# myshell-ai/OpenVoice

Measured on NVIDIA H100. Metric: audio_seconds_per_second, higher is better.
Workload: dtype f32 (3xFP16 split-precision tensor-core convs with fp32 accumulation, fp32 FFMA elsewhere)

## Files before the change

### include/ovc.h

```cpp
#ifndef OVC_B200_H
#define OVC_B200_H

#include <stddef.h>
#include <stdint.h>

#ifdef __cplusplus
extern "C" {
#endif

#define OVC_ABI_VERSION 17

#if defined(__GNUC__)
#define OVC_API __attribute__((visibility("default")))
#else
#define OVC_API
#endif

enum {
  OVC_OK = 0,
  OVC_ERR_INVALID = -1,
  OVC_ERR_CUDA = -2,
  OVC_ERR_STATE = -3,
  OVC_ERR_MISSING = -4,
  OVC_ERR_NOMEM = -5
};
// ... 154 lines not shown
                                      float* d_stats, int32_t* d_cum, float* d_g, int64_t* d_y_lengths, void* stream);
OVC_API int ovc_tts_decode_windows_tokens(ovc_ctx* ctx, const float* stats, const int32_t* cum, const float* g,
                                          const int64_t* y_lengths, int N, int T, const int64_t* row, const int64_t* frame0,
                                          const int64_t* len, int W, int Wmax, const uint64_t* seed, const int64_t* stream,
                                          const float* noise_scale, float* o, float* z_p, void* cuda_stream);

OVC_API int ovc_set_precision(ovc_ctx* ctx, int mode);

#define OVC_OPT_TTS_SIMPLE 2
#define OVC_OPT_GRAPH 3
#define OVC_OPT_PDL 5
#define OVC_OPT_BRANCHES 7
#define OVC_OPT_PAIR 8
#define OVC_OPT_PAIR_OCC 9
#define OVC_OPT_STAGED_EPI 10
OVC_API int ovc_set_option(ovc_ctx* ctx, int key, int value);

OVC_API int ovc_last_launch_count(const ovc_ctx* ctx);

OVC_API int ovc_graph_replays(const ovc_ctx* ctx);

OVC_API int ovc_profile_enable(ovc_ctx* ctx, int enable);
OVC_API int ovc_profile_read(ovc_ctx* ctx, double* ms, int64_t* launches, double* flops, double* bytes);
OVC_API int ovc_profile_detail(ovc_ctx* ctx, int max, char* names, double* ms, double* flops, double* bytes,
                               int* family);

OVC_API int ovc_debug_enable(ovc_ctx* ctx, int enable);
OVC_API int ovc_debug_fetch(ovc_ctx* ctx, const char* name, float* host_out, size_t max_floats,
                    int64_t* shape4 );

// ... 5 lines not shown
```

### openvoice_b200/_native.py

```python
from __future__ import annotations

import ctypes as C
import os
from typing import Dict, Iterable, Optional, Tuple

_HERE = os.path.dirname(os.path.abspath(__file__))
LIB_PATH = os.path.join(_HERE, "libovc_b200.so")

ABI_VERSION = 17
EXPORTS = (
    "ovc_abi_version", "ovc_last_error", "ovc_create", "ovc_destroy", "ovc_load_tensor",
    "ovc_finalize_weights", "ovc_workspace_floats", "ovc_voice_conversion", "ovc_last_launch_count",
    "ovc_profile_enable", "ovc_profile_read", "ovc_profile_detail", "ovc_debug_enable", "ovc_debug_fetch",
    "ovc_spectrogram", "ovc_convert_waveform", "ovc_set_precision", "ovc_reference_encoder",
    "ovc_tts_info", "ovc_tts_encode", "ovc_tts_decode", "ovc_set_option", "ovc_graph_replays",
    "ovc_reference_encoder_ragged", "ovc_resample", "ovc_resample_span", "ovc_voice_conversion_items",
    "ovc_convert_waveform_items", "ovc_tts_encode_items", "ovc_tts_decode_items", "ovc_philox_normals",
    "ovc_tts_encode_state", "ovc_tts_decode_windows", "ovc_spectrogram_ring", "ovc_splice",
    "ovc_tts_encode_state_rows", "ovc_tts_state_rows", "ovc_resample_plan", "ovc_resample_rings",
    "ovc_voice_conversion_frames", "ovc_convert_waveform_frames", "ovc_tone_track_expand",
    "ovc_tts_encode_g", "ovc_tts_encode_state_tokens", "ovc_tts_decode_windows_tokens", "ovc_tts_encode_state_rows_tokens",
    "ovc_tts_state_rows_tokens", "ovc_reference_encoder_stream", "ovc_reference_encoder_stream_state_floats",
    "ovc_generate_frames",
)
# ... 259 lines not shown
            _check(self.lib, rc, f"ovc_load_tensor({k})")
            (ignored if rc == 1 else used).append(k)
        self.finalized = False
        return used, ignored

    def finalize(self):
        _check(self.lib, self.lib.ovc_finalize_weights(self.handle), "ovc_finalize_weights")
        self.finalized = True

    def set_precision(self, mode: str):
        m = PRECISIONS[mode]
        _check(self.lib, self.lib.ovc_set_precision(self.handle, m), "ovc_set_precision")
        self.precision = mode

    def set_option(self, key: str, value: int):
        k = {"tts_simple": 2, "graph": 3, "pdl": 5, "branches": 7, "pair": 8, "pair_occ": 9, "staged_epi": 10}[key]
        _check(self.lib, self.lib.ovc_set_option(self.handle, k, int(value)), "ovc_set_option")

    def voice_conversion(self, spec, lengths, g_src, g_tgt, noise=None, tau: float = 0.3, seed: int = 0,
                         ragged: bool = False, latents: bool = True, stream=None, items: Optional[dict] = None, out=None):
        import torch
        assert spec.is_cuda and spec.dtype == torch.float32 and spec.is_contiguous()
        assert lengths.is_cuda and lengths.dtype == torch.int64 and lengths.is_contiguous()
        B, S, T = spec.shape
        gs, fs = se_arg(g_src, B, self.hp.gin_channels, T, "g_src")
        gt, ft = se_arg(g_tgt, B, self.hp.gin_channels, T, "g_tgt")
        if noise is not None:
            noise = noise.contiguous().float()
            assert tuple(noise.shape) == (B, self.hp.inter_channels, T)
        hop = self.hp.hop_length
        if out is not None:
# ... 486 lines not shown
```

### openvoice_b200/csrc/ovc_lib.cu

```cuda
#include <cuda_runtime.h>

#include <algorithm>
#include <cmath>
#include <cstdarg>
#include <cstdio>
#include <cstdlib>
#include <cstring>
#include <map>
#include <string>
#include <vector>

#include "../../include/ovc.h"
#include "ovc_convpack.h"
#include "ovc_small.cuh"
#include "ovc_tcconv.cuh"
#include "ovc_tts.cuh"
#include "ovc_refenc.cuh"
#include "ovc_resample.cuh"
#include "ovc_splice.h"
#include "ovc_variants.h"

namespace ovc {

static thread_local std::string g_err;
// ... 135 lines not shown
  WNLayers flow_wn[4];
  ConvLayer dec_pre, dec_ups[4];
  ConvLayer rb_c1[12][3], rb_c2[12][3];
  TcLayer tc_c1[12][3], tc_c2[12][3], tc_ups[4], tc_pre;
  float* d_tcw = nullptr;
  std::vector<float> h_tcw;
  int precision = 0;
  bool tts_simple = false;
  bool use_graph = true;
  int use_pdl = 2;
  bool use_branches = true;
  int par_frames = 512;
  bool use_pair = true;
  bool use_pair_occ = true;
  bool use_staged_epi = true;
  bool pair_occ2_ok[TCN_N_OCC2] = {};
  cudaStream_t br_stream[2] = {nullptr, nullptr};
  cudaEvent_t br_ev[4] = {nullptr, nullptr, nullptr, nullptr};
  size_t post_w_off = 0;
  size_t cond_w_off = 0, cond_b_off = 0;
  int* d_cond_wrow = nullptr;
  int* d_cond_sel = nullptr;
  int cond_rows_out = 0;
  int cond_off_enc = 0, cond_off_fsrc = 0, cond_off_ftgt = 0, cond_off_dec = 0;
  int cond_off_enc_tc = 0, cond_off_fsrc_tc = 0, cond_off_ftgt_tc = 0;
  int* d_cond_cols[2][3] = {};
  int cond_pf_cols[2][3] = {};
  int cond_pf_off[2][3][4] = {};

  float2* d_tw = nullptr;
// ... 427 lines not shown
  if (c->d_w) { cudaFree(c->d_w); c->d_w = nullptr; }
  c->w_floats = c->h_w.size();
  CK(cudaMalloc(&c->d_w, c->w_floats * sizeof(float)));
  CK(cudaMemcpy(c->d_w, c->h_w.data(), c->w_floats * sizeof(float), cudaMemcpyHostToDevice));
  if (c->d_tcw) { cudaFree(c->d_tcw); c->d_tcw = nullptr; }
  CK(cudaMalloc(&c->d_tcw, c->h_tcw.size() * sizeof(float)));
  CK(cudaMemcpy(c->d_tcw, c->h_tcw.data(), c->h_tcw.size() * sizeof(float), cudaMemcpyHostToDevice));
  c->h_tcw.clear();
  c->h_tcw.shrink_to_fit();
  for (int TN : {128, 64, 32})
    for (bool staged : {false, true}) {
      const TcKernel k = tc_conv_kernel(TN, staged), p = tc_pair_kernel(TN, TcPairOcc(), staged);
      CK(cudaFuncSetAttribute(k.fn, cudaFuncAttributeMaxDynamicSharedMemorySize, (int)k.smem));
      CK(cudaFuncSetAttribute(p.fn, cudaFuncAttributeMaxDynamicSharedMemorySize, (int)p.smem));
    }
  for (int i = 0; i < TCN_N_OCC2; ++i) {
    const TcKernel k = tc_pair_kernel(kTcPairOcc2[i].C, kTcPairOcc2[i].o);
    CK(cudaFuncSetAttribute(k.fn, cudaFuncAttributeMaxDynamicSharedMemorySize, (int)k.smem));
    int blocks = 0;
    CK(cudaOccupancyMaxActiveBlocksPerMultiprocessor(&blocks, k.fn, k.threads, k.smem));
    c->pair_occ2_ok[i] = blocks >= 2;
    if (blocks < 2)
      fprintf(stderr, "ovc: the C = %d conv-pair kernel with %d operand buffer(s) fits %d CTA(s) per SM, not 2; its pairs run "
              "one CTA per SM\n", kTcPairOcc2[i].C, kTcPairOcc2[i].o.nabuf, blocks);
  }
  if (c->d_cond_wrow) cudaFree(c->d_cond_wrow);
  if (c->d_cond_sel) cudaFree(c->d_cond_sel);
  CK(cudaMalloc(&c->d_cond_wrow, wrow.size() * sizeof(int)));
  CK(cudaMalloc(&c->d_cond_sel, sel.size() * sizeof(int)));
  CK(cudaMemcpy(c->d_cond_wrow, wrow.data(), wrow.size() * sizeof(int), cudaMemcpyHostToDevice));
// ... 135 lines not shown
  CK(cudaEventRecord(c->ev[c->ev_used], r.st));
  return OVC_OK;
}
static int prof_end(Run& r, int variant, int family, double flops, double bytes, int tag = 0) {
  ovc_ctx* c = r.c;
  if (!c->prof) return OVC_OK;
  CK(cudaEventRecord(c->ev[c->ev_used + 1], r.st));
  c->ev_used += 2;
  c->ev_flops.push_back(flops);
  c->ev_bytes.push_back(bytes);
  c->ev_variant.push_back(variant);
  c->ev_family.push_back(family);
  c->ev_tag.push_back(tag);
  return OVC_OK;
}
enum { V_TCPAIR128 = -14, V_TCPAIR64 = -12, V_TCPAIR32 = -13, V_TC128 = -1, V_TC64 = -2, V_TC32 = -3, V_TRANSPOSE = -4, V_TTS_DENSE = -5, V_TTS_LN = -6, V_TTS_SCORES = -7,
       V_TTS_ATTN = -8, V_TTS_DW = -9, V_TTS_SPLINE = -10, V_TTS_MISC = -11 };
static const char* variant_name(int v) {
  if (v >= 0) return kInfo[v].name;
  switch (v) {
    case V_TCPAIR128: return "PAIR_N128";
    case V_TCPAIR64: return "PAIR_N64";
    case V_TCPAIR32: return "PAIR_N32";
    case V_TC128: return "TC3_N128";
    case V_TC64: return "TC3_N64";
    case V_TC32: return "TC3_N32";
    case V_TTS_DENSE: return "TTS_DENSE32";
    case V_TTS_LN: return "TTS_LAYERNORM";
    case V_TTS_SCORES: return "TTS_SCORES";
    case V_TTS_ATTN: return "TTS_ATTN_OUT";
    case V_TTS_DW: return "TTS_DWCONV";
    case V_TTS_SPLINE: return "TTS_SPLINE";
    case V_TTS_MISC: return "TTS_MISC";
    default: return "TRANSPOSE";
  }
// ... 119 lines not shown
    TRY(launch(r, wn.in[i], a, T));
    ConvArgs b{};
    b.x = acts; b.x_bs = bs; b.x_pitch = P;
    b.bias = r.c->d_w + wn.rs[i].b_off; b.bias_bs = 0;
    b.y = x; b.y_bs = bs; b.y_pitch = P;
    b.s = skip; b.s_bs = bs; b.s_pitch = P;
    b.lens_in = r.lens; b.lens_out = r.lens; b.mul_in = 1; b.mul_out = 1;
    b.slope = 1.f;
    b.split = (i < n - 1) ? 192 : 0;
    b.flags = (i == 0) ? F_FIRST : 0;
    TRY(launch(r, wn.rs[i], b, T));
  }
  return OVC_OK;
}

static int run_wn_tc(Run& r, const WNLayers& wn, float* x, float* skip, float* acts, float* x_cl, float* skip_cl,
                     const CondRef& cond_tc) {
  const int P = r.P, T = r.Tmax;
  const int n = (int)wn.tc_in.size();
  TRY(launch_transpose(r, x, x_cl, 192, P));
  for (int i = 0; i < n; ++i) {
    TcExtra g;
    g.epi = 1; g.bias = cond_tc.p + (size_t)i * 384; g.bias_bs = cond_tc.bs; g.bias_ts = cond_tc.ts; g.y_ld = 192;
    g.use_lens_frames = true;
    TRY(launch_tc(r, wn.tc_in[i], x_cl, acts, nullptr, T, 1, 1.f, 1.f, 0, 0, g));
    TcExtra q;
    q.epi = 2; q.s = skip_cl; q.split = (i < n - 1) ? 192 : 0; q.first = (i == 0); q.y_ld = 192; q.use_lens_frames = true;
    TRY(launch_tc(r, wn.tc_rs[i], acts, x_cl, nullptr, T, 1, 1.f, 1.f, 0, 0, q));
  }
  TRY(launch_transpose(r, skip_cl, skip, P, 192));
  return OVC_OK;
}

static int run_flow(Run& r, const WsLayout& W, float* ws, bool reverse, const CondRef& cond) {
  ovc_ctx* c = r.c;
  const int P = r.P, T = r.Tmax;
// ... 103 lines not shown
  }
  e->launches = c->launches;
  CK(cudaGraphLaunch(e->exec, st));
  c->graph_replays++;
  return OVC_OK;
}

static int set_call_params(ovc_ctx* c, uint64_t seed, float tau, const ItemParams& items, cudaStream_t st) {
  if (!c->d_callp) CK(cudaMalloc(&c->d_callp, sizeof(CallParams)));
  set_call_params_kernel<<<1, 1, 0, st>>>(c->d_callp, seed, tau, items);
  CK(cudaGetLastError());
  return OVC_OK;
}
static uintptr_t option_bits(const ovc_ctx* c) {
  return (uintptr_t)c->precision | ((uintptr_t)c->use_pdl << 15) | ((uintptr_t)c->use_branches << 14) | ((uintptr_t)c->use_pair << 17) |
         ((uintptr_t)c->use_pair_occ << 18) | ((uintptr_t)c->use_staged_epi << 19);
}

static int ensure_ws(ovc_ctx* c, const WsLayout& W, int B, int Tmax, cudaStream_t st) {
  if (W.total <= c->ws_floats) return OVC_OK;
  CK(cudaStreamSynchronize(st));
  drop_graphs(c);
  if (c->d_ws) CK(cudaFree(c->d_ws));
  c->d_ws = nullptr;
  c->ws_floats = 0;
  cudaError_t e = cudaMalloc(&c->d_ws, W.total * sizeof(float));
  if (e != cudaSuccess) {
    cudaGetLastError();
    return fail(OVC_ERR_NOMEM, "workspace of %.2f GB for B=%d Tmax=%d does not fit: %s", W.total * 4e-9, B, Tmax,
                cudaGetErrorString(e));
  }
// ... 1095 lines not shown
}

int ovc_set_option(ovc_ctx* c, int key, int value) {
  if (!c) return fail(OVC_ERR_INVALID, "null context");
  switch (key) {
    case OVC_OPT_TTS_SIMPLE: c->tts_simple = value != 0; return OVC_OK;
    case OVC_OPT_GRAPH: c->use_graph = value != 0; return OVC_OK;
    case OVC_OPT_PDL:
      if (value < 0 || value > 2) return fail(OVC_ERR_INVALID, "pdl must be 0, 1 or 2");
      c->use_pdl = value;
      return OVC_OK;
    case OVC_OPT_BRANCHES: c->use_branches = value != 0; return OVC_OK;
    case OVC_OPT_PAIR: c->use_pair = value != 0; return OVC_OK;
    case OVC_OPT_PAIR_OCC: c->use_pair_occ = value != 0; return OVC_OK;
    case OVC_OPT_STAGED_EPI: c->use_staged_epi = value != 0; return OVC_OK;
    default: return fail(OVC_ERR_INVALID, "unknown option %d", key);
  }
}

int ovc_last_launch_count(const ovc_ctx* c) { return c ? c->launches : 0; }

int ovc_graph_replays(const ovc_ctx* c) { return c ? c->graph_replays : 0; }

int ovc_profile_enable(ovc_ctx* c, int enable) {
  if (!c) return fail(OVC_ERR_INVALID, "null context");
  c->prof = enable != 0;
  c->ev_used = 0;
  c->ev_flops.clear();
  c->ev_bytes.clear();
  c->ev_variant.clear();
// ... 76 lines not shown
```

### openvoice_b200/csrc/ovc_tcconv.cuh

```cuda
#pragma once
#include "ovc_conv.cuh"
#include "ovc_tc.cuh"
#include "ovc_tcpack.h"

namespace ovc {

struct TcConvArgs {
  const float* x; long long x_bs;
  const uint16_t* w;
  const float* bias; long long bias_bs;
  float* y; long long y_bs; int y_ld;
  const float* r;
  float* s; long long s_bs;
  int epi;
  int split; int first;
  const long long* lens; int tmax; int mul;
  const long long* lens_x; int has_lens_x;
  int Cin; int Ntot; int K; int DIL;
  float slope; float scale; int accumulate;
  int passes;
  const uint16_t* w2; const float* bias2;
  long long bias_ts;
};

__device__ __forceinline__ void pdl_launch_dependents() { asm volatile("griddepcontrol.launch_dependents;" ::: "memory"); }
__device__ __forceinline__ void pdl_wait() { asm volatile("griddepcontrol.wait;" ::: "memory"); }

__device__ __forceinline__ void mbar_arrive(uint64_t* bar) {
  asm volatile("mbarrier.arrive.shared::cta.b64 _, [%0];" ::"r"(smem_u32(bar)) : "memory");
}
__device__ __forceinline__ void named_bar_sync(int id, int threads) {
  asm volatile("bar.sync %0, %1;" ::"r"(id), "r"(threads) : "memory");
}
__device__ __forceinline__ void named_bar_arrive(int id, int threads) {
  asm volatile("bar.arrive %0, %1;" ::"r"(id), "r"(threads) : "memory");
}

template <int TN>
__device__ __forceinline__ float tc_result(const float (&d)[TN], bool two, int j) {
  return two ? fmaf(d[TN / 2 + j], tc::kLoInv, d[j]) : d[j];
}

template <int TN, bool PF, class V>
__device__ __forceinline__ void tc_epilogue_body(const TcConvArgs& a, V v_at, int b, int t0, int n0, int lim, int row_a) {
  const int csub = (threadIdx.x & 3) * 2;
  float* yb = a.y + (size_t)b * a.y_bs;
  const float* rb = a.r ? a.r + (size_t)b * a.y_bs : nullptr;
  float* sb = a.s ? a.s + (size_t)b * a.s_bs : nullptr;
  const int ta = t0 + row_a, tb = ta + 8;
  const bool oka = ta < lim, okb = tb < lim;
  const float* bias_a = a.bias + (size_t)b * a.bias_bs + (PF ? (size_t)min(ta, a.tmax - 1) * a.bias_ts : 0);
  const float* bias_b = a.bias + (size_t)b * a.bias_bs + (PF ? (size_t)min(tb, a.tmax - 1) * a.bias_ts : 0);
#pragma unroll
  for (int c0 = 0; c0 < TN; c0 += 32) {
    float v[16];
#pragma unroll
    for (int i = 0; i < 16; ++i) v[i] = v_at(c0 / 2 + i);
#pragma unroll
    for (int g = 0; g < 4; ++g) {
// ... 21 lines not shown
          ob.x = yc.x + ob.x; ob.y = yc.y + ob.y;
        }
        if (a.scale != 1.f) { oa.x *= a.scale; oa.y *= a.scale; ob.x *= a.scale; ob.y *= a.scale; }
        if (oka) *reinterpret_cast<float2*>(ypa + 8 * g) = oa;
        if (okb) *reinterpret_cast<float2*>(ypb + 8 * g) = ob;
      }
    } else if (a.epi == 1) {
      float* ypa = yb + (size_t)ta * a.y_ld + ((n0 + c0) >> 1) + csub;
      float* ypb = yb + (size_t)tb * a.y_ld + ((n0 + c0) >> 1) + csub;
#pragma unroll
      for (int g = 0; g < 2; ++g) {
        const float2 oa = make_float2(tanhf(v[4 * g]) * sigmoidf_acc(v[4 * (g + 2)]),
                                      tanhf(v[4 * g + 1]) * sigmoidf_acc(v[4 * (g + 2) + 1]));
        const float2 ob = make_float2(tanhf(v[4 * g + 2]) * sigmoidf_acc(v[4 * (g + 2) + 2]),
                                      tanhf(v[4 * g + 3]) * sigmoidf_acc(v[4 * (g + 2) + 3]));
        if (oka) *reinterpret_cast<float2*>(ypa + 8 * g) = oa;
        if (okb) *reinterpret_cast<float2*>(ypb + 8 * g) = ob;
      }
    } else {
      const int col = n0 + c0;
      const bool to_x = col < a.split;
      const bool add = to_x || !a.first;
      float* dst = (to_x ? yb + col : sb + (col - a.split)) + csub;
#pragma unroll
      for (int g = 0; g < 4; ++g) {
        float2 oa = make_float2(v[4 * g], v[4 * g + 1]), ob = make_float2(v[4 * g + 2], v[4 * g + 3]);
        if (add) {
          const float2 qa = oka ? *reinterpret_cast<const float2*>(dst + (size_t)ta * a.y_ld + 8 * g) : make_float2(0.f, 0.f);
          const float2 qb = okb ? *reinterpret_cast<const float2*>(dst + (size_t)tb * a.y_ld + 8 * g) : make_float2(0.f, 0.f);
          oa = make_float2(qa.x + oa.x, qa.y + oa.y);
          ob = make_float2(qb.x + ob.x, qb.y + ob.y);
        }
        if (oka) *reinterpret_cast<float2*>(dst + (size_t)ta * a.y_ld + 8 * g) = oa;
        if (okb) *reinterpret_cast<float2*>(dst + (size_t)tb * a.y_ld + 8 * g) = ob;
      }
    }
  }
}

template <int TN, class V>
__device__ __forceinline__ void tc_epilogue_v(const TcConvArgs& a, V v_at, int b, int t0, int n0, int lim, int row_a) {
  if (a.bias_ts) tc_epilogue_body<TN, true>(a, v_at, b, t0, n0, lim, row_a);
  else tc_epilogue_body<TN, false>(a, v_at, b, t0, n0, lim, row_a);
}

template <int TN>
__device__ __forceinline__ void tc_epilogue(const TcConvArgs& a, const float (&d)[TN], int b, int t0, int n0, int lim, int row_a) {
  const bool two = a.passes == 3;
  tc_epilogue_v<TN>(a, [&](int j) { return tc_result<TN>(d, two, j); }, b, t0, n0, lim, row_a);
}
__device__ __forceinline__ TcConvArgs tc_pair_epilogue_args(const TcConvArgs& a, int TN) {
  TcConvArgs e = a;
  e.y_ld = TN; e.r = a.x; e.bias = a.bias2; e.bias_bs = 0; e.bias_ts = 0; e.epi = 0;
  return e;
}

template <int TN>
__device__ __forceinline__ void tc_mma_step(float (&d)[TN], uint64_t a_hi, uint64_t a_lo, uint64_t b, bool three, bool first) {
  float (&lo)[TN / 2] = *reinterpret_cast<float(*)[TN / 2]>(&d[TN / 2]);
  float (&hi)[TN / 2] = *reinterpret_cast<float(*)[TN / 2]>(&d[0]);
  tc::Wgmma<TN>::mma(hi, a_hi, b, first ? 0 : 1);
  if (three) {
    tc::Wgmma<TN>::mma(lo, a_hi, b + TN, first ? 0 : 1);
    tc::Wgmma<TN>::mma(lo, a_lo, b, 1);
  }
}

constexpr int TCN_THREADS = 384;
constexpr int TCN_NCT = 96;

template <int TN, bool PAIR, int OCC = 1, int NAB = 2, bool STAGED = false>
struct TcnCfg {
  static_assert(!PAIR || TN == 32 || TN == 64 || TN == 128, "conv pairs: C = 32, 64 or 128");
  static_assert(OCC == 1 || (PAIR && TN <= 64), "two CTAs per SM: C = 32 / 64 pairs");
  static_assert(!STAGED || (TN == 128 && OCC == 1), "staged epilogue: TN = 128, one CTA per SM");
  static constexpr int THREADS = STAGED ? TCN_THREADS + 128 : TCN_THREADS;
  static constexpr int KCH = 32, NKC = KCH / 8;
  static constexpr int ROWS = 194;
  static constexpr int ROWS2 = TCN_ROWS2;
  static constexpr int NABUF = NAB;
  static constexpr int RING = PAIR ? tc_pair_ring(TN, OCC, NAB) : tc_ring_slots(TN, PAIR);
  static constexpr int SLOT_BYTES = 2 * 2 * TN * 16;
  static constexpr int A_BUF_BYTES = 2 * NKC * ROWS * 16;
  static constexpr int A2_BYTES = PAIR ? 2 * (TN / 8) * ROWS2 * 16 : 0;
// ... 36 lines not shown
  constexpr uint32_t BYTES = Cfg::SLOT_BYTES;

  if (tid == 0) {
    for (int i = 0; i < NABUF; ++i) { mbar_init(&a_full[i], TCN_NCT); mbar_init(&a_empty[i], 2); }
    for (int i = 0; i < RING; ++i) { mbar_init(&b_full[i], 1); mbar_init(&b_empty[i], 2); }
    if (STAGED) { mbar_init(s_full, 256); mbar_init(s_empty, 128); }
    fence_mbar_init();
  }
  if (PAIR) {
    for (int i = tid; i < Cfg::A2_BYTES / 16; i += Cfg::THREADS) reinterpret_cast<uint4*>(a2buf)[i] = make_uint4(0u, 0u, 0u, 0u);
    asm volatile("fence.proxy.async.shared::cta;" ::: "memory");
  }
  __syncthreads();
  pdl_launch_dependents();
  if (warp != 0) pdl_wait();

#define TCN_FOR_TILES                                                                                   \
  for (int tile = blockIdx.x; tile < total; tile += gridDim.x) {                                        \
    const int b = tile / n_tt, t0 = (tile % n_tt) * R;                                                  \
    const int lim = (a.lens ? (int)min((long long)a.tmax, a.lens[b]) : a.tmax) * a.mul;                 \
    const int lim_x = a.has_lens_x ? (int)min((long long)a.tmax, a.lens_x[b]) * a.mul : lim;            \
    (void)lim_x;                                                                                        \
    if (t0 >= lim) continue;

  if (warp < 4) {
    tc::regs_dealloc<Cfg::PROD_REGS>();
    if (warp == 0) {
      if (lane == 0) {
        const unsigned char* wt = reinterpret_cast<const unsigned char*>(a.w) + (size_t)blockIdx.y * n_slots * BYTES;
        if (resident) {
          for (int it = 0; it < n_w; ++it) {
            const unsigned char* src = it < n_slots ? wt + (size_t)it * BYTES
                                                    : reinterpret_cast<const unsigned char*>(a.w2) + (size_t)(it - n_slots) * BYTES;
            mbar_expect_tx(&b_full[it], BYTES);
            tma_bulk_g2s(bring + it * BYTES, src, BYTES, &b_full[it]);
          }
          for (int it = 0; it < n_w; ++it) mbar_wait(&b_full[it], 0u);
        } else {
// ... 193 lines not shown
          }
        }
        tc::wgmma_commit();
        tc::wgmma_wait<0>();
        tc::fence_regs(d);
        if (leader && prev >= 0) mbar_arrive(&b_empty[prev]);
        if constexpr (STAGED) {
          named_bar_sync(3, 256);
          stage_tile();
        } else {
          tc_epilogue<TN>(tc_pair_epilogue_args(a, TN), d, b, t0, 0, min(lim, t0 + R), row_a);
        }
      }
    }
  }
#undef TCN_FOR_TILES
}

struct TcKernel {
  void (*fn)(TcConvArgs, int, int) = nullptr;
  size_t smem = 0;
  int threads = 0;
};
using TcPairKernel = TcKernel;
template <int TN, bool PAIR, int OCC = 1, int NAB = 2, bool STAGED = false>
inline TcKernel tc_kernel() {
  using Cfg = TcnCfg<TN, PAIR, OCC, NAB, STAGED>;
  return {tcconv_kernel<TN, PAIR, OCC, NAB, STAGED>, Cfg::SMEM_BYTES, Cfg::THREADS};
}
inline bool tc_stage_pays(int K, int passes) { return passes * K >= 15; }
inline TcKernel tc_conv_kernel(int TN, bool staged) {
  if (TN == 128) return staged ? tc_kernel<128, false, 1, 2, true>() : tc_kernel<128, false>();
  if (TN == 64) return tc_kernel<64, false>();
  if (TN == 32) return tc_kernel<32, false>();
  return {};
}
inline TcKernel tc_pair_kernel(int C, TcPairOcc o, bool staged = false) {
  if (o.occ == 1 && o.nabuf == 2) {
    if (C == 128) return staged ? tc_kernel<128, true, 1, 2, true>() : tc_kernel<128, true>();
    if (C == 64) return tc_kernel<64, true>();
    if (C == 32) return tc_kernel<32, true>();
  } else if (o.occ == 2) {
    if (C == 32 && o.nabuf == 2) return tc_kernel<32, true, 2, 2>();
    if (C == 32 && o.nabuf == 1) return tc_kernel<32, true, 2, 1>();
    if (C == 64 && o.nabuf == 1) return tc_kernel<64, true, 2, 1>();
  }
  return {};
}
constexpr int TCN_N_OCC2 = 3;
constexpr struct { int C; TcPairOcc o; } kTcPairOcc2[TCN_N_OCC2] = {{32, {2, 2}}, {32, {2, 1}}, {64, {2, 1}}};

template <int C>
__global__ void __launch_bounds__(256) conv_post_cl_kernel(const float* __restrict__ x, long long x_bs,
                                                           const float* __restrict__ w, float* __restrict__ y,
                                                           long long y_bs, int y_len, const long long* lens, int tmax,
                                                           int mul) {
  constexpr int TB = 256, ROWS = TB + 6, LD = ROWS + 3;
  __shared__ float ws[7][C];
  __shared__ float xs[C][LD];
  for (int i = threadIdx.x; i < C * 7; i += blockDim.x) ws[i % 7][i / 7] = w[i];
  const int b = blockIdx.y;
// ... 47 lines not shown
```

### openvoice_b200/csrc/ovc_tcpack.h

```cpp
#pragma once
#include <cuda_fp16.h>
#include <stddef.h>
#include <stdint.h>

#include <algorithm>

namespace ovc {

constexpr int TCN_HMAX = 25;
constexpr int TCN_ROWS2 = 146;

constexpr int tc_ring_slots(int TN, bool pair) {
  return pair ? (TN == 32 ? 44 : TN == 64 ? 24 : 12) : (TN == 32 ? 22 : 12);
}

struct TcGeom {
  int Cin = 0, Ntot = 0, K = 0, DIL = 1, TN = 0;
};

inline int tc_tile_n(int Ntot, int Cin, int K, int DIL) {
  if (Ntot <= 0 || Cin <= 0 || K <= 0 || DIL <= 0) return 0;
  if (Ntot % 32 || Cin % 32 || (K - 1) / 2 * DIL > TCN_HMAX) return 0;
  return Ntot % 128 == 0 ? 128 : (Ntot % 64 == 0 ? 64 : 32);
}
// ... 41 lines not shown
}

inline bool tc_pair_fits(const TcGeom& T1, const TcGeom& T2) {
  if (!(T1.TN == 32 || T1.TN == 64)) return false;
  const int ring = tc_ring_slots(T1.TN, true);
  return T1.Ntot == T1.TN && T1.Cin == T1.TN && T2.Ntot == T1.TN && T2.Cin == T1.TN && T2.TN == T1.TN && T2.K == T1.K &&
         T2.DIL == 1 && (T1.K - 1) / 2 * T1.DIL <= TCN_HMAX && 2 * (T1.Cin / 16) * T1.K <= ring && T1.K <= 5;
}

inline bool tc_pair_fuses(const TcGeom& T1, const TcGeom& T2) {
  if (!(T1.TN == 32 || T1.TN == 64 || T1.TN == 128)) return false;
  return T1.Ntot == T1.TN && T1.Cin == T1.TN && T2.Ntot == T1.TN && T2.Cin == T1.TN && T2.TN == T1.TN && T2.K == T1.K &&
         T2.DIL == 1 && (T1.K - 1) / 2 * T1.DIL <= TCN_HMAX && 128 + 2 * ((T2.K - 1) / 2) <= TCN_ROWS2;
}

struct TcGrid {
  int n_tt = 0, total = 0, grid_x = 0, ncol = 0;
};
inline TcGrid tc_grid(int t_len, int B, int Ntot, int TN, int sm_count, int grid_div) {
  TcGrid g;
  g.n_tt = (t_len + 127) / 128;
  g.total = g.n_tt * B;
  g.ncol = Ntot / TN;
  const int per_col = std::max(1, sm_count / g.ncol / std::max(1, grid_div));
  g.grid_x = std::min(g.total, per_col);
  return g;
}
inline TcGrid tc_pair_grid(int t_len, int B, int K, int sm_count, int occ = 1) {
  TcGrid g;
  const int R = 128 - (K - 1);
// ... 30 lines not shown
```

Before: 2381.

## Fuse WaveNet gated conv and res/skip projection into one tensor-core kernel

Adds a warp-specialized kernel that computes the K=5 gate convolution for each 128-frame tile, applies tanh·sigmoid gating in the epilogue, and stores the activations as split fp16 hi/lo in shared memory. The 1x1 res/skip projection then reads those activations straight from shared memory, and the residual add reads the input buffer. This removes the global round-trip of the activation tensor and one launch per WaveNet layer, at the cost of a large shared-memory footprint that limits occupancy to one block per SM. The fused path is on by default but only runs when the tile count is at least the SM count.

```diff
diff --git a/include/ovc.h b/include/ovc.h
--- a/include/ovc.h
+++ b/include/ovc.h
@@ -8,7 +8,7 @@
 extern "C" {
 #endif
 
-#define OVC_ABI_VERSION 17
+#define OVC_ABI_VERSION 18
 
 #if defined(__GNUC__)
 #define OVC_API __attribute__((visibility("default")))
@@ -193,6 +193,7 @@
 #define OVC_OPT_PAIR 8
 #define OVC_OPT_PAIR_OCC 9
 #define OVC_OPT_STAGED_EPI 10
+#define OVC_OPT_WN_FUSE 11
 OVC_API int ovc_set_option(ovc_ctx* ctx, int key, int value);
 
 OVC_API int ovc_last_launch_count(const ovc_ctx* ctx);
diff --git a/openvoice_b200/_native.py b/openvoice_b200/_native.py
--- a/openvoice_b200/_native.py
+++ b/openvoice_b200/_native.py
@@ -7,7 +7,7 @@
 _HERE = os.path.dirname(os.path.abspath(__file__))
 LIB_PATH = os.path.join(_HERE, "libovc_b200.so")
 
-ABI_VERSION = 17
+ABI_VERSION = 18
 EXPORTS = (
     "ovc_abi_version", "ovc_last_error", "ovc_create", "ovc_destroy", "ovc_load_tensor",
     "ovc_finalize_weights", "ovc_workspace_floats", "ovc_voice_conversion", "ovc_last_launch_count",
@@ -297,7 +297,7 @@
         self.precision = mode
 
     def set_option(self, key: str, value: int):
-        k = {"tts_simple": 2, "graph": 3, "pdl": 5, "branches": 7, "pair": 8, "pair_occ": 9, "staged_epi": 10}[key]
+        k = {"tts_simple": 2, "graph": 3, "pdl": 5, "branches": 7, "pair": 8, "pair_occ": 9, "staged_epi": 10, "wn_fuse": 11}[key]
         _check(self.lib, self.lib.ovc_set_option(self.handle, k, int(value)), "ovc_set_option")
 
     def voice_conversion(self, spec, lengths, g_src, g_tgt, noise=None, tau: float = 0.3, seed: int = 0,
diff --git a/openvoice_b200/csrc/ovc_lib.cu b/openvoice_b200/csrc/ovc_lib.cu
--- a/openvoice_b200/csrc/ovc_lib.cu
+++ b/openvoice_b200/csrc/ovc_lib.cu
@@ -173,6 +173,7 @@
   bool use_pair = true;
   bool use_pair_occ = true;
   bool use_staged_epi = true;
+  bool use_wn_fuse = true;
   bool pair_occ2_ok[TCN_N_OCC2] = {};
   cudaStream_t br_stream[2] = {nullptr, nullptr};
   cudaEvent_t br_ev[4] = {nullptr, nullptr, nullptr, nullptr};
@@ -630,6 +631,10 @@
       CK(cudaFuncSetAttribute(k.fn, cudaFuncAttributeMaxDynamicSharedMemorySize, (int)k.smem));
       CK(cudaFuncSetAttribute(p.fn, cudaFuncAttributeMaxDynamicSharedMemorySize, (int)p.smem));
     }
+  for (int TN2 : {128, 64}) {
+    const TcKernel k = tc_wn_kernel(TN2);
+    CK(cudaFuncSetAttribute(k.fn, cudaFuncAttributeMaxDynamicSharedMemorySize, (int)k.smem));
+  }
   for (int i = 0; i < TCN_N_OCC2; ++i) {
     const TcKernel k = tc_pair_kernel(kTcPairOcc2[i].C, kTcPairOcc2[i].o);
     CK(cudaFuncSetAttribute(k.fn, cudaFuncAttributeMaxDynamicSharedMemorySize, (int)k.smem));
@@ -795,11 +800,12 @@
   c->ev_tag.push_back(tag);
   return OVC_OK;
 }
-enum { V_TCPAIR128 = -14, V_TCPAIR64 = -12, V_TCPAIR32 = -13, V_TC128 = -1, V_TC64 = -2, V_TC32 = -3, V_TRANSPOSE = -4, V_TTS_DENSE = -5, V_TTS_LN = -6, V_TTS_SCORES = -7,
+enum { V_TCWN = -15, V_TCPAIR128 = -14, V_TCPAIR64 = -12, V_TCPAIR32 = -13, V_TC128 = -1, V_TC64 = -2, V_TC32 = -3, V_TRANSPOSE = -4, V_TTS_DENSE = -5, V_TTS_LN = -6, V_TTS_SCORES = -7,
        V_TTS_ATTN = -8, V_TTS_DW = -9, V_TTS_SPLINE = -10, V_TTS_MISC = -11 };
 static const char* variant_name(int v) {
   if (v >= 0) return kInfo[v].name;
   switch (v) {
+    case V_TCWN: return "TCWN";
     case V_TCPAIR128: return "PAIR_N128";
     case V_TCPAIR64: return "PAIR_N64";
     case V_TCPAIR32: return "PAIR_N32";
@@ -949,12 +955,46 @@
   return OVC_OK;
 }
 
+static int launch_wn(Run& r, const TcLayer& G, const TcLayer& RS, const float* x_in, float* x_out, float* skip,
+                     const CondRef& cond, int first) {
+  const int P = r.P, T = r.Tmax;
+  TcConvArgs a{};
+  a.x = x_in; a.x_bs = 192LL * P;
+  a.w = reinterpret_cast<const uint16_t*>(r.c->d_tcw + G.w_off);
+  a.bias = cond.p; a.bias_bs = cond.bs; a.bias_ts = cond.ts;
+  a.w2 = reinterpret_cast<const uint16_t*>(r.c->d_tcw + RS.w_off); a.bias2 = r.c->d_tcw + RS.b_off;
+  a.y = x_out; a.y_bs = 192LL * P; a.y_ld = 192;
+  a.r = x_in;
+  a.s = skip; a.s_bs = a.y_bs;
+  a.split = RS.Ntot - 192; a.first = first;
+  a.lens = r.lens; a.tmax = T; a.mul = 1;
+  a.Cin = G.Cin; a.Ntot = G.Ntot; a.K = G.K; a.DIL = G.DIL;
+  a.slope = 1.f; a.scale = 1.f;
+  a.passes = r.c->precision == 2 ? 1 : 3;
+  if (!tc_wn_fuses(G, RS)) return fail(OVC_ERR_INVALID, "WaveNet layer %d -> %d / %d does not fit the fused layer kernel", G.Cin, G.Ntot, RS.Ntot);
+  const TcKernel k = tc_wn_kernel(RS.TN);
+  const TcGrid g = tc_grid(T, r.B, 128, 128, r.c->sm_count, 1);
+  TRY(prof_begin(r));
+  CK(launch_ex(k.fn, dim3((unsigned)g.grid_x, 1, 1), k.threads, k.smem, r.st, r.c->use_pdl != 0, a, g.n_tt, g.total));
+  CK(cudaGetLastError());
+  r.c->launches++;
+  const double units = (double)r.B * T;
+  TRY(prof_end(r, V_TCWN, 0, 2.0 * 192 * (G.Ntot * G.K + RS.Ntot) * units, 4.0 * 192 * (3 + (first ? 0 : 1)) * units));
+  return OVC_OK;
+}
+
 static int run_wn_tc(Run& r, const WNLayers& wn, float* x, float* skip, float* acts, float* x_cl, float* skip_cl,
                      const CondRef& cond_tc) {
   const int P = r.P, T = r.Tmax;
   const int n = (int)wn.tc_in.size();
   TRY(launch_transpose(r, x, x_cl, 192, P));
+  const bool fuse = r.c->use_wn_fuse && tc_wn_pays(tc_grid(T, r.B, 128, 128, r.c->sm_count, 1).total, r.c->sm_count);
   for (int i = 0; i < n; ++i) {
+    if (fuse) {
+      float* x_in = i % 2 ? acts : x_cl;
+      TRY(launch_wn(r, wn.tc_in[i], wn.tc_rs[i], x_in, i % 2 ? x_cl : acts, skip_cl, cond_tc.at(i * 384), i == 0));
+      continue;
+    }
     TcExtra g;
     g.epi = 1; g.bias = cond_tc.p + (size_t)i * 384; g.bias_bs = cond_tc.bs; g.bias_ts = cond_tc.ts; g.y_ld = 192;
     g.use_lens_frames = true;
@@ -1088,7 +1128,7 @@
 }
 static uintptr_t option_bits(const ovc_ctx* c) {
   return (uintptr_t)c->precision | ((uintptr_t)c->use_pdl << 15) | ((uintptr_t)c->use_branches << 14) | ((uintptr_t)c->use_pair << 17) |
-         ((uintptr_t)c->use_pair_occ << 18) | ((uintptr_t)c->use_staged_epi << 19);
+         ((uintptr_t)c->use_pair_occ << 18) | ((uintptr_t)c->use_staged_epi << 19) | ((uintptr_t)c->use_wn_fuse << 20);
 }
 
 static int ensure_ws(ovc_ctx* c, const WsLayout& W, int B, int Tmax, cudaStream_t st) {
@@ -2214,6 +2254,7 @@
     case OVC_OPT_PAIR: c->use_pair = value != 0; return OVC_OK;
     case OVC_OPT_PAIR_OCC: c->use_pair_occ = value != 0; return OVC_OK;
     case OVC_OPT_STAGED_EPI: c->use_staged_epi = value != 0; return OVC_OK;
+    case OVC_OPT_WN_FUSE: c->use_wn_fuse = value != 0; return OVC_OK;
     default: return fail(OVC_ERR_INVALID, "unknown option %d", key);
   }
 }
diff --git a/openvoice_b200/csrc/ovc_tcconv.cuh b/openvoice_b200/csrc/ovc_tcconv.cuh
--- a/openvoice_b200/csrc/ovc_tcconv.cuh
+++ b/openvoice_b200/csrc/ovc_tcconv.cuh
@@ -36,13 +36,16 @@
   asm volatile("bar.arrive %0, %1;" ::"r"(id), "r"(threads) : "memory");
 }
 
+constexpr int TCWN_ACT_HALF_BYTES = (192 / 8) * 128 * 16;
+
 template <int TN>
 __device__ __forceinline__ float tc_result(const float (&d)[TN], bool two, int j) {
   return two ? fmaf(d[TN / 2 + j], tc::kLoInv, d[j]) : d[j];
 }
 
-template <int TN, bool PF, class V>
-__device__ __forceinline__ void tc_epilogue_body(const TcConvArgs& a, V v_at, int b, int t0, int n0, int lim, int row_a) {
+template <int TN, bool PF, bool WN, class V>
+__device__ __forceinline__ void tc_epilogue_body(const TcConvArgs& a, V v_at, int b, int t0, int n0, int lim, int row_a,
+                                                 unsigned char* acts) {
   const int csub = (threadIdx.x & 3) * 2;
   float* yb = a.y + (size_t)b * a.y_bs;
   const float* rb = a.r ? a.r + (size_t)b * a.y_bs : nullptr;
@@ -94,6 +97,19 @@
                                       tanhf(v[4 * g + 1]) * sigmoidf_acc(v[4 * (g + 2) + 1]));
         const float2 ob = make_float2(tanhf(v[4 * g + 2]) * sigmoidf_acc(v[4 * (g + 2) + 2]),
                                       tanhf(v[4 * g + 3]) * sigmoidf_acc(v[4 * (g + 2) + 3]));
+        if constexpr (WN) {
+          const int off = ((((n0 + c0) >> 4) + g) * 128 + row_a) * 16 + csub * 2;
+          const float2 za = oka ? oa : make_float2(0.f, 0.f), zb = okb ? ob : make_float2(0.f, 0.f);
+          const __half2 ha = __floats2half2_rn(za.x, za.y), hb = __floats2half2_rn(zb.x, zb.y);
+          const float2 fa = __half22float2(ha), fb = __half22float2(hb);
+          *reinterpret_cast<__half2*>(acts + off) = ha;
+          *reinterpret_cast<__half2*>(acts + off + 8 * 16) = hb;
+          *reinterpret_cast<__half2*>(acts + TCWN_ACT_HALF_BYTES + off) =
+              __floats2half2_rn((za.x - fa.x) * tc::kLoScale, (za.y - fa.y) * tc::kLoScale);
+          *reinterpret_cast<__half2*>(acts + TCWN_ACT_HALF_BYTES + off + 8 * 16) =
+              __floats2half2_rn((zb.x - fb.x) * tc::kLoScale, (zb.y - fb.y) * tc::kLoScale);
+          continue;
+        }
         if (oka) *reinterpret_cast<float2*>(ypa + 8 * g) = oa;
         if (okb) *reinterpret_cast<float2*>(ypb + 8 * g) = ob;
       }
@@ -102,12 +118,13 @@
       const bool to_x = col < a.split;
       const bool add = to_x || !a.first;
       float* dst = (to_x ? yb + col : sb + (col - a.split)) + csub;
+      const float* src = WN && to_x ? rb + col + csub : dst;
 #pragma unroll
       for (int g = 0; g < 4; ++g) {
         float2 oa = make_float2(v[4 * g], v[4 * g + 1]), ob = make_float2(v[4 * g + 2], v[4 * g + 3]);
         if (add) {
-          const float2 qa = oka ? *reinterpret_cast<const float2*>(dst + (size_t)ta * a.y_ld + 8 * g) : make_float2(0.f, 0.f);
-          const float2 qb = okb ? *reinterpret_cast<const float2*>(dst + (size_t)tb * a.y_ld + 8 * g) : make_float2(0.f, 0.f);
+          const float2 qa = oka ? *reinterpret_cast<const float2*>(src + (size_t)ta * a.y_ld + 8 * g) : make_float2(0.f, 0.f);
+          const float2 qb = okb ? *reinterpret_cast<const float2*>(src + (size_t)tb * a.y_ld + 8 * g) : make_float2(0.f, 0.f);
           oa = make_float2(qa.x + oa.x, qa.y + oa.y);
           ob = make_float2(qb.x + ob.x, qb.y + ob.y);
         }
@@ -118,16 +135,18 @@
   }
 }
 
-template <int TN, class V>
-__device__ __forceinline__ void tc_epilogue_v(const TcConvArgs& a, V v_at, int b, int t0, int n0, int lim, int row_a) {
-  if (a.bias_ts) tc_epilogue_body<TN, true>(a, v_at, b, t0, n0, lim, row_a);
-  else tc_epilogue_body<TN, false>(a, v_at, b, t0, n0, lim, row_a);
-}
-
-template <int TN>
-__device__ __forceinline__ void tc_epilogue(const TcConvArgs& a, const float (&d)[TN], int b, int t0, int n0, int lim, int row_a) {
+template <int TN, bool WN = false, class V>
+__device__ __forceinline__ void tc_epilogue_v(const TcConvArgs& a, V v_at, int b, int t0, int n0, int lim, int row_a,
+                                              unsigned char* acts = nullptr) {
+  if (a.bias_ts) tc_epilogue_body<TN, true, WN>(a, v_at, b, t0, n0, lim, row_a, acts);
+  else tc_epilogue_body<TN, false, WN>(a, v_at, b, t0, n0, lim, row_a, acts);
+}
+
+template <int TN, bool WN = false>
+__device__ __forceinline__ void tc_epilogue(const TcConvArgs& a, const float (&d)[TN], int b, int t0, int n0, int lim, int row_a,
+                                            unsigned char* acts = nullptr) {
   const bool two = a.passes == 3;
-  tc_epilogue_v<TN>(a, [&](int j) { return tc_result<TN>(d, two, j); }, b, t0, n0, lim, row_a);
+  tc_epilogue_v<TN, WN>(a, [&](int j) { return tc_result<TN>(d, two, j); }, b, t0, n0, lim, row_a, acts);
 }
 __device__ __forceinline__ TcConvArgs tc_pair_epilogue_args(const TcConvArgs& a, int TN) {
   TcConvArgs e = a;
@@ -148,6 +167,49 @@
 
 constexpr int TCN_THREADS = 384;
 constexpr int TCN_NCT = 96;
+
+template <int ROWS>
+__device__ __forceinline__ void tc_convert_chunk(const TcConvArgs& a, const float* xb, int r0, int q, int lim_x, int items,
+                                                 unsigned char* ah, int pt) {
+  constexpr int NKC = 4, KCH = 32;
+  unsigned char* al = ah + NKC * ROWS * 16;
+  constexpr int PB = 2;
+  for (int i0 = pt; i0 < items; i0 += TCN_NCT * PB) {
+    float4 v0[PB], v1[PB];
+#pragma unroll
+    for (int u = 0; u < PB; ++u) {
+      const int i = i0 + TCN_NCT * u;
+      const int row = i >> 2, kc = i & 3;
+      const int t = r0 + row;
+      v0[u] = make_float4(0.f, 0.f, 0.f, 0.f);
+      v1[u] = v0[u];
+      if (i < items && t >= 0 && t < lim_x) {
+        const float4* src = reinterpret_cast<const float4*>(xb + (size_t)t * a.Cin + q * KCH + kc * 8);
+        v0[u] = src[0];
+        v1[u] = src[1];
+      }
+    }
+#pragma unroll
+    for (int u = 0; u < PB; ++u) {
+      const int i = i0 + TCN_NCT * u;
+      if (i >= items) break;
+      const int row = i >> 2, kc = i & 3;
+      uint4 hi, lo;
+      tc::split_f16x8(v0[u], v1[u], a.slope, hi, lo);
+      *reinterpret_cast<uint4*>(ah + (kc * ROWS + row) * 16) = hi;
+      *reinterpret_cast<uint4*>(al + (kc * ROWS + row) * 16) = lo;
+    }
+  }
+  asm volatile("fence.proxy.async.shared::cta;" ::: "memory");
+}
+
+#define TCN_FOR_TILES                                                                                   \
+  for (int tile = blockIdx.x; tile < total; tile += gridDim.x) {                                        \
+    const int b = tile / n_tt, t0 = (tile % n_tt) * R;                                                  \
+    const int lim = (a.lens ? (int)min((long long)a.tmax, a.lens[b]) : a.tmax) * a.mul;                 \
+    const int lim_x = a.has_lens_x ? (int)min((long long)a.tmax, a.lens_x[b]) * a.mul : lim;            \
+    (void)lim_x;                                                                                        \
+    if (t0 >= lim) continue;
 
 template <int TN, bool PAIR, int OCC = 1, int NAB = 2, bool STAGED = false>
 struct TcnCfg {
@@ -214,14 +276,6 @@
   __syncthreads();
   pdl_launch_dependents();
   if (warp != 0) pdl_wait();
-
-#define TCN_FOR_TILES                                                                                   \
-  for (int tile = blockIdx.x; tile < total; tile += gridDim.x) {                                        \
-    const int b = tile / n_tt, t0 = (tile % n_tt) * R;                                                  \
-    const int lim = (a.lens ? (int)min((long long)a.tmax, a.lens[b]) : a.tmax) * a.mul;                 \
-    const int lim_x = a.has_lens_x ? (int)min((long long)a.tmax, a.lens_x[b]) * a.mul : lim;            \
-    (void)lim_x;                                                                                        \
-    if (t0 >= lim) continue;
 
   if (warp < 4) {
     tc::regs_dealloc<Cfg::PROD_REGS>();
@@ -445,8 +499,181 @@
       }
     }
   }
+}
+
+template <int TN2>
+struct TcwnCfg {
+  static_assert(TN2 == 128 || TN2 == 64, "res/skip column tile: 128 (384 rows) or 64 (192 rows)");
+  static constexpr int H = 192, NQ = H / 32, K = 5, NPASS = 3;
+  static constexpr int GATE_SLOTS = (H / 16) * K;
+  static constexpr int RS_SLOTS = H / 16;
+  static constexpr int ROWS = TcnCfg<128, false>::ROWS;
+  static constexpr int NABUF = 2, RING = 10;
+  static constexpr int SLOT_BYTES = 2 * 2 * 128 * 16;
+  static constexpr int SLOT2_BYTES = 2 * 2 * TN2 * 16;
+  static constexpr int A_BUF_BYTES = TcnCfg<128, false>::A_BUF_BYTES;
+  static constexpr int ACT_BYTES = 2 * TCWN_ACT_HALF_BYTES;
+  static constexpr size_t SMEM_BYTES = 1024 + NABUF * A_BUF_BYTES + ACT_BYTES + RING * SLOT_BYTES;
+  static_assert(SMEM_BYTES <= 232448, "shared memory budget");
+  static_assert((2 * NABUF + 2 * RING) * 8 <= 1024, "barrier area");
+  static constexpr int PROD_REGS = 56, MMA_REGS = 224;
+  static_assert(128 * PROD_REGS + 256 * MMA_REGS <= 65536, "register budget");
+};
+
+template <int TN2>
+__global__ void __launch_bounds__(TCN_THREADS, 1) tcwn_kernel(const TcConvArgs a, int n_tt, int total) {
+  using Cfg = TcwnCfg<TN2>;
+  constexpr int ROWS = Cfg::ROWS, NABUF = Cfg::NABUF, RING = Cfg::RING, NQ = Cfg::NQ, K = Cfg::K, NPASS = Cfg::NPASS;
+  constexpr int R = 128;
+  extern __shared__ __align__(128) unsigned char smem_raw[];
+  uint64_t* bars = reinterpret_cast<uint64_t*>(smem_raw);
+  uint64_t *a_full = bars, *a_empty = bars + NABUF, *b_full = a_empty + NABUF, *b_empty = b_full + RING;
+  unsigned char* abuf = smem_raw + 1024;
+  unsigned char* acts = abuf + NABUF * Cfg::A_BUF_BYTES;
+  unsigned char* bring = acts + Cfg::ACT_BYTES;
+
+  const int tid = threadIdx.x, lane = tid & 31;
+  const int warp = __shfl_sync(0xffffffffu, tid >> 5, 0);
+
+  if (tid == 0) {
+    for (int i = 0; i < NABUF; ++i) { mbar_init(&a_full[i], TCN_NCT); mbar_init(&a_empty[i], 2); }
+    for (int i = 0; i < RING; ++i) { mbar_init(&b_full[i], 1); mbar_init(&b_empty[i], 2); }
+    fence_mbar_init();
+  }
+  __syncthreads();
+  pdl_launch_dependents();
+  if (warp != 0) pdl_wait();
+
+  if (warp < 4) {
+    tc::regs_dealloc<Cfg::PROD_REGS>();
+    if (warp == 0) {
+      if (lane == 0) {
+        const unsigned char* w1 = reinterpret_cast<const unsigned char*>(a.w);
+        const unsigned char* w2 = reinterpret_cast<const unsigned char*>(a.w2);
+        int slot = 0;
+        uint32_t phase = 1;
+        const auto put = [&](const unsigned char* src, uint32_t bytes) {
+          mbar_wait(&b_empty[slot], phase);
+          mbar_expect_tx(&b_full[slot], bytes);
+          tma_bulk_g2s(bring + slot * Cfg::SLOT_BYTES, src, bytes, &b_full[slot]);
+          if (++slot == RING) { slot = 0; phase ^= 1; }
+        };
+        TCN_FOR_TILES
+          (void)b;
+          for (int it = 0; it < NPASS * Cfg::GATE_SLOTS; ++it) put(w1 + (size_t)it * Cfg::SLOT_BYTES, Cfg::SLOT_BYTES);
+          for (int it = 0; it < NPASS * Cfg::RS_SLOTS; ++it) put(w2 + (size_t)it * Cfg::SLOT2_BYTES, Cfg::SLOT2_BYTES);
+        }
+      }
+    } else {
+      int buf = 0;
+      uint32_t ephase = 1;
+      TCN_FOR_TILES
+        const float* xb = a.x + (size_t)b * a.x_bs;
+        for (int p = 0; p < NPASS; ++p)
+          for (int q = 0; q < NQ; ++q) {
+            mbar_wait(&a_empty[buf], ephase);
+            tc_convert_chunk<ROWS>(a, xb, t0 - (K - 1) / 2, q, lim_x, ((128 + K - 1 + 7) & ~7) * 4,
+                                   abuf + buf * Cfg::A_BUF_BYTES, tid - 32);
+            mbar_arrive(&a_full[buf]);
+            if (++buf == NABUF) { buf = 0; ephase ^= 1; }
+          }
+      }
+    }
+  } else {
+    tc::regs_alloc<Cfg::MMA_REGS>();
+    const int wg = (warp >> 2) - 1;
+    const bool leader = (tid & 127) == 0;
+    const int row_a = 64 * wg + 16 * (warp & 3) + (lane >> 2);
+    constexpr uint32_t LBO_A = ROWS * 16, LBO_ACT = 128 * 16, SBO = 128;
+    constexpr uint32_t A_LO16 = (4 * ROWS * 16) >> 4, ACT_LO16 = TCWN_ACT_HALF_BYTES >> 4, SLOT16 = Cfg::SLOT_BYTES >> 4;
+    const uint64_t a_proto = tc::make_desc(0, LBO_A, SBO), act_proto = tc::make_desc(0, LBO_ACT, SBO);
+    const uint64_t b_ring = tc::make_desc(0, 2 * 128 * 16, SBO) + (tc::smem_addr(bring) >> 4);
+    const uint64_t b2_ring = tc::make_desc(0, 2 * TN2 * 16, SBO) + (tc::smem_addr(bring) >> 4);
+    const uint64_t act_base = act_proto + ((tc::smem_addr(acts) + 64 * wg * 16) >> 4);
+    const bool three = a.passes == 3;
+    TcConvArgs ge = a;
+    ge.epi = 1;
+    TcConvArgs re = a;
+    re.epi = 2; re.bias = a.bias2; re.bias_bs = 0; re.bias_ts = 0;
+    float d[128];
+#pragma unroll
+    for (int i = 0; i < 128; ++i) d[i] = 0.f;
+    constexpr bool OWN = TN2 != 128;
+    float e[OWN ? TN2 : 1];
+    float (&d2)[TN2] = *reinterpret_cast<float(*)[TN2]>(OWN ? &e[0] : &d[0]);
+    int slot = 0, buf = 0;
+    uint32_t bphase = 0, aphase = 0;
+    int prev = -1;
+    const auto release_prev = [&]() {
+      if (leader && prev >= 0) mbar_arrive(&b_empty[prev]);
+      prev = slot;
+      if (++slot == RING) { slot = 0; bphase ^= 1; }
+    };
+    TCN_FOR_TILES
+      (void)lim_x;
+      if constexpr (OWN) {
+#pragma unroll
+        for (int i = 0; i < 128; ++i) d[i] = 0.f;
+      }
+#pragma unroll 1
+      for (int p = 0; p < NPASS; ++p) {
+        bool first = true;
+        for (int q = 0; q < NQ; ++q) {
+          mbar_wait(&a_full[buf], aphase);
+          tc::fence_regs(d);
+          tc::wgmma_fence();
+          prev = -1;
+          for (int j = 0; j < 2; ++j) {
+            uint64_t a_cur = a_proto + ((tc::smem_addr(abuf + buf * Cfg::A_BUF_BYTES) + 64 * wg * 16 + 2 * j * LBO_A) >> 4);
+            for (int tap = 0; tap < K; ++tap) {
+              mbar_wait(&b_full[slot], bphase);
+              tc_mma_step<128>(d, a_cur, a_cur + A_LO16, b_ring + (uint32_t)slot * SLOT16, three, first);
+              tc::wgmma_commit();
+              tc::wgmma_wait<1>();
+              release_prev();
+              first = false;
+              a_cur += 1;
+            }
+          }
+          tc::wgmma_wait<0>();
+          tc::fence_regs(d);
+          if (leader) {
+            mbar_arrive(&b_empty[prev]);
+            mbar_arrive(&a_empty[buf]);
+          }
+          if (++buf == NABUF) { buf = 0; aphase ^= 1; }
+        }
+        if (p == 0) named_bar_sync(1 + wg, 128);
+        tc_epilogue<128, true>(ge, d, b, t0, 128 * p, lim, row_a, acts);
+      }
+      asm volatile("fence.proxy.async.shared::cta;" ::: "memory");
+      named_bar_sync(1 + wg, 128);
+      if constexpr (OWN) {
+#pragma unroll
+        for (int i = 0; i < TN2; ++i) d2[i] = 0.f;
+      }
+#pragma unroll 1
+      for (int p = 0; p < NPASS; ++p) {
+        tc::fence_regs(d2);
+        tc::wgmma_fence();
+        prev = -1;
+        for (int kk = 0; kk < Cfg::RS_SLOTS; ++kk) {
+          const uint64_t a_cur = act_base + 2 * kk * (LBO_ACT >> 4);
+          mbar_wait(&b_full[slot], bphase);
+          tc_mma_step<TN2>(d2, a_cur, a_cur + ACT_LO16, b2_ring + (uint32_t)slot * SLOT16, three, kk == 0);
+          tc::wgmma_commit();
+          tc::wgmma_wait<1>();
+          release_prev();
+        }
+        tc::wgmma_wait<0>();
+        tc::fence_regs(d2);
+        if (leader) mbar_arrive(&b_empty[prev]);
+        tc_epilogue<TN2, true>(re, d2, b, t0, TN2 * p, lim, row_a);
+      }
+    }
+  }
+}
 #undef TCN_FOR_TILES
-}
 
 struct TcKernel {
   void (*fn)(TcConvArgs, int, int) = nullptr;
@@ -476,6 +703,11 @@
     if (C == 32 && o.nabuf == 1) return tc_kernel<32, true, 2, 1>();
     if (C == 64 && o.nabuf == 1) return tc_kernel<64, true, 2, 1>();
   }
+  return {};
+}
+inline TcKernel tc_wn_kernel(int TN2) {
+  if (TN2 == 128) return {tcwn_kernel<128>, TcwnCfg<128>::SMEM_BYTES, TCN_THREADS};
+  if (TN2 == 64) return {tcwn_kernel<64>, TcwnCfg<64>::SMEM_BYTES, TCN_THREADS};
   return {};
 }
 constexpr int TCN_N_OCC2 = 3;
diff --git a/openvoice_b200/csrc/ovc_tcpack.h b/openvoice_b200/csrc/ovc_tcpack.h
--- a/openvoice_b200/csrc/ovc_tcpack.h
+++ b/openvoice_b200/csrc/ovc_tcpack.h
@@ -79,6 +79,13 @@
          T2.DIL == 1 && (T1.K - 1) / 2 * T1.DIL <= TCN_HMAX && 128 + 2 * ((T2.K - 1) / 2) <= TCN_ROWS2;
 }
 
+inline bool tc_wn_fuses(const TcGeom& gate, const TcGeom& rs) {
+  return gate.Cin == 192 && gate.Ntot == 384 && gate.K == 5 && gate.DIL == 1 && gate.TN == 128 && rs.Cin == 192 &&
+         rs.K == 1 && rs.DIL == 1 && ((rs.Ntot == 384 && rs.TN == 128) || (rs.Ntot == 192 && rs.TN == 64));
+}
+
+inline bool tc_wn_pays(int tiles, int sm_count) { return tiles >= sm_count; }
+
 struct TcGrid {
   int n_tt = 0, total = 0, grid_x = 0, ncol = 0;
 };
```

Measured after the change: 2450, median of 6. 2.9% higher.
